# DelphinusLab/halo2-gpu-specific

Measured on AMD Instinct MI355X. Metric: NTT Fr-ops/s @ k=24 (forward+inverse 2^24 BN254 Fr NTT; MSM G1-adds/s under 'msm'), higher is better.
Workload: dtype u32x8 (254-bit Montgomery, integer)

## Files before the change

halo2-gpu-specific_amd/csrc/ntt.hip:

```cpp
#include <algorithm>
#include <cstdlib>
#include <memory>
#include <utility>

#include "common.hpp"
#include "ntt.hpp"
#include "ntt_pass.hpp"

namespace h2 {

void ntt_split(uint32_t log_n, std::vector<uint32_t>& bits) {
    bits.clear();
    if (log_n == 0) return;
    const uint32_t rem = log_n % 8, q = log_n / 8;
    static const bool nine = !(getenv("H2_NTT_NINE") && atoi(getenv("H2_NTT_NINE")) == 0);
    if (nine && q >= rem && (rem == 1 || (rem == 2 && log_n <= 18))) {
        for (uint32_t p = 0; p < q - rem; p++) bits.push_back(8);
        for (uint32_t p = 0; p < rem; p++) bits.push_back(9);
        return;
    }
    if (rem) bits.push_back(rem);
    for (uint32_t p = 0; p < q; p++) bits.push_back(8);
}

// ... 11 lines not shown
    sh.fixed = sh.radix4 && B == 8 && log_c == 2 && threads == 256;
    return sh;
}

std::vector<NttPass> ntt_schedule(uint32_t log_n) {
    std::vector<uint32_t> bits;
    ntt_split(log_n, bits);
    if (bits.empty()) bits.push_back(0);
    std::vector<NttPass> sched;
    uint32_t consumed = 0;
    for (size_t p = 0; p < bits.size(); p++) {
        NttPass ps{};
        ps.B = bits[p];
        ps.t_log = consumed;
        ps.s_log = log_n - consumed - ps.B;
        ps.last = p + 1 == bits.size();
        ps.shape = pass_shape(log_n, ps.B, ps.last ? ps.t_log : ps.s_log);
        sched.push_back(ps);
        consumed += ps.B;
    }
    return sched;
}

static uint32_t pass_zskip(uint32_t L, const NttPass& ps, uint32_t in_len) {
    static const bool no_zskip = getenv("H2_NTT_NO_ZSKIP") != nullptr;
    if (ps.t_log != 0 || ps.last || !in_len || in_len >= (1u << L) || (in_len & (in_len - 1)) != 0 || no_zskip) return 0;
    uint32_t z = 0;
    while ((in_len << z) < (1u << L)) z++;
    return z < ps.B ? z : ps.B;
}

static NttKernel pass_kernel(const NttPass& ps, uint32_t zskip) {
    if (!ps.shape.radix4) return NK_R2;
    const bool dp = !ps.last;
    if (ps.shape.fixed && zskip == 0) return dp ? NK_PASS8_DP : NK_PASS8;
    return dp ? NK_R4_DP : NK_R4;
}

size_t ntt_shape_query(uint32_t log_n, uint32_t in_log, uint32_t* out, size_t cap) {
    if (log_n == 0) return 0;
    const std::vector<NttPass> sched = ntt_schedule(log_n);
    for (size_t p = 0; p < sched.size() && p < cap; p++) {
        const NttPass& ps = sched[p];
        const uint32_t zskip = pass_zskip(log_n, ps, 1u << in_log);
        const uint32_t row[7] = {ps.B, ps.shape.log_c, ps.shape.threads, ps.shape.radix4, ps.shape.fixed, zskip,
                                 (uint32_t)pass_kernel(ps, zskip)};
        for (int i = 0; i < 7; i++) out[7 * p + i] = row[i];
    }
    return sched.size();
}

static std::string plan_key(uint32_t log_n, const uint64_t omega[4]) {
    char buf[128];
    snprintf(buf, sizeof buf, "%u:%016llx%016llx%016llx%016llx", log_n, (unsigned long long)omega[3],
             (unsigned long long)omega[2], (unsigned long long)omega[1], (unsigned long long)omega[0]);
    return buf;
}

static std::string fr_key(const Fr& v) {
    char buf[72];
    snprintf(buf, sizeof buf, "%08x%08x%08x%08x%08x%08x%08x%08x", v.l[7], v.l[6], v.l[5], v.l[4], v.l[3], v.l[2], v.l[1], v.l[0]);
    return buf;
}

Fr fr_from_u64x4(const uint64_t v[4]) {
    Fr r;
    for (int i = 0; i < 4; i++) {
        r.l[2 * i] = (uint32_t)v[i];
        r.l[2 * i + 1] = (uint32_t)(v[i] >> 32);
// ... 150 lines not shown
        ntt_fill_scaled(block.p, pl->tw_hi, d, cnt, stream);
        return block.publish(cnt * sizeof(Fr), stream);
    };
    return table_get(pl->cache, pl->scaled_hi, fr_key(d), build, [](std::vector<Fr*>&) {});
}

NttTablePin ntt_scale_table(NttPlan* pl, const Fr& g, const Fr* d, hipStream_t stream) {
    auto build = [&]() -> NttTable {
        const uint32_t n = 1u << pl->log_n;
        const uint32_t lo_count = n < (1u << LO_BITS) ? n : (1u << LO_BITS);
        const uint32_t hi_count = pl->log_n > LO_BITS ? (n >> LO_BITS) : 1u;
        const size_t bytes = ((size_t)(1u << LO_BITS) + hi_count) * sizeof(Fr);
        TableBlock block;
        H2_HIP(hipMalloc(&block.p, bytes));
        Fr* const hi = block.p + (1u << LO_BITS);
        ntt_fill_pow(block.p, g, 1u, lo_count, 0u, stream);
        ntt_fill_pow(hi, g, 1u << LO_BITS, hi_count, 0u, stream);
        if (d) ntt_fill_scaled(hi, hi, *d, hi_count, stream);
        return block.publish(bytes, stream);
    };
    auto admit = [&](std::vector<Fr*>& gone) {
        while (pl->scale_tabs.size() >= NttPlan::SCALE_TABS_MAX) {
            const auto lru = lru_idle(pl->scale_tabs);
            if (lru == pl->scale_tabs.end()) break;
            gone.push_back(lru->second.ptr);
            pl->scale_tabs.erase(lru);
        }
    };
    return table_get(pl->cache, pl->scale_tabs, d ? fr_key(g) + '*' + fr_key(*d) : fr_key(g) + '.', build, admit);
}

static void free_plan(NttPlan* pl) {
    if (pl->tables) (void)hipFree(pl->tables);
    for (const Fr* t : pl->tw_direct)
        if (t) (void)hipFree(const_cast<Fr*>(t));
    for (NttTableMap* map : {&pl->scaled_hi, &pl->scale_tabs, &pl->last_direct})
        for (auto& kv : *map) (void)hipFree(kv.second.ptr);
    delete pl;
}

static size_t plan_bytes(NttPlan* pl, bool* pinned = nullptr) {
    size_t bytes = pl->table_bytes;
    for (NttTableMap* map : {&pl->scaled_hi, &pl->scale_tabs, &pl->last_direct})
        for (auto& kv : *map) {
            bytes += kv.second.bytes;
            if (pinned && kv.second.users != 0) *pinned = true;
        }
    return bytes;
}

size_t ntt_plan_bytes(DeviceCtx* ctx) {
    NttCache* c = ctx->shared->ntt;
    std::lock_guard<std::mutex> g(c->mu);
    size_t bytes = 0;
    for (auto& kv : c->plans) bytes += plan_bytes(kv.second);
    return bytes;
}

void ntt_release_idle_plans(DeviceCtx* ctx) {
    NttCache* c = ctx->shared->ntt;
    std::vector<NttPlan*> gone;
    {
        std::lock_guard<std::mutex> g(c->mu);
        for (auto it = c->plans.begin(); it != c->plans.end();) {
            NttPlan* pl = it->second;
            bool busy = pl->users.load() != 0;
            plan_bytes(pl, &busy);
// ... 24 lines not shown
    };
    {
        std::lock_guard<std::mutex> g(c->mu);
        if (NttPlan* found = pin()) return PlanRef(found);
    }

    std::unique_ptr<NttPlan, void (*)(NttPlan*)> pl(new NttPlan(), free_plan);
    pl->cache = c;
    pl->log_n = log_n;
    pl->sched = ntt_schedule(log_n);
    const Fr w = pl->w = fr_from_u64x4(omega);
    const uint32_t n = 1u << log_n;
    const uint32_t lo_count = n < (1u << LO_BITS) ? n : (1u << LO_BITS);
    const uint32_t hi_count = log_n > LO_BITS ? (n >> LO_BITS) : 0;
    auto bfly_entries = [](const NttPass& ps) { return ((1u << ps.B) >> 1) * (ps.shape.radix4 ? 2u : 1u); };
    auto chunk_entries = [](const NttPass& ps) { return ps.shape.fixed ? ((1u << ps.B) >> 1) * TW_CHUNK_FR : 0u; };
    size_t total = lo_count + hi_count;
    for (const NttPass& ps : pl->sched) total += bfly_entries(ps) + chunk_entries(ps);
    H2_HIP(hipMalloc(&pl->tables, total * sizeof(Fr)));
    pl->table_bytes = total * sizeof(Fr);
    pl->tw_lo = pl->tables;
    pl->tw_hi = pl->tables + lo_count;
    ntt_fill_pow(pl->tables, w, 1u, lo_count, 0u, stream);
    ntt_fill_pow(pl->tables + lo_count, w, 1u << LO_BITS, hi_count, 0u, stream);
    Fr* next = pl->tables + lo_count + hi_count;
    for (const NttPass& ps : pl->sched) {
        const uint32_t half = (1u << ps.B) >> 1, form = ps.shape.radix4 ? 1u : 0u;
        ntt_fill_pow(next, w, n >> ps.B, half, form, stream);
        pl->tw_bfly.push_back(next);
        next += bfly_entries(ps);
        if (ps.shape.fixed) ntt_fill_pow(next, w, n >> ps.B, half, 2u, stream);
        pl->tw_chunk.push_back(ps.shape.fixed ? next : nullptr);
        next += chunk_entries(ps);
        Fr* direct = nullptr;
        if (ps.t_log != 0 && !ps.last && ps.B + ps.t_log <= 16) {
            const uint32_t cnt = 1u << (ps.B + ps.t_log);
            const size_t bytes = (size_t)cnt * sizeof(Fr) * (form ? 2 : 1);
            H2_HIP(hipMalloc(&direct, bytes));
            pl->table_bytes += bytes;
        }
        pl->tw_direct.push_back(direct);
        if (direct) ntt_fill_direct(direct, w, ps.t_log, ps.s_log, log_n, 1u << (ps.B + ps.t_log), form, stream);
    }
    H2_HIP(hipGetLastError());
    H2_HIP(hipStreamSynchronize(stream));
    std::lock_guard<std::mutex> g(c->mu);
    if (NttPlan* raced = pin()) return PlanRef(raced);
    c->plans[key] = pl.get();
    pl.release();
    return PlanRef(pin());
}

static void set_scale3(PassArgs& a, const Fr* pre3, const Fr* post3) {
    a.has_pre3 = pre3 != nullptr;
    a.has_post3 = post3 != nullptr;
    a.post3_uniform = post3 && fp_eq(post3[0], post3[1]) && fp_eq(post3[0], post3[2]);
    for (int i = 0; i < 3; i++) {
        if (pre3) a.pre3[i] = pre3[i];
        if (post3) a.post3[i] = post3[i];
    }
}

void ntt_run(DeviceCtx* ctx, NttPlan* pl, const Fr* src, Fr* dst, Fr* tmp, uint32_t in_len, const Fr* pre3,
             const Fr* post3, hipStream_t stream, const Fr* scale_tab, uint32_t scale_mode) {
    ntt_run_many(ctx, pl, &src, &dst, &tmp, 1, in_len, pre3, post3, stream, scale_tab, scale_mode);
}

static PassArgs pass_args(const NttPlan* pl, size_t p, const Fr* const* srcs, Fr* const* dsts, Fr* const* tmps, uint32_t cnt,
                          uint32_t in_len, const Fr* pre3, const Fr* post3, const Fr* scale_tab, uint32_t scale_mode) {
    const NttPass& ps = pl->sched[p];
    const bool first = p == 0, chain = pl->sched.size() >= 2;
    PassArgs a{};
    a.in = first ? srcs[0] : tmps[0];
    a.out = ps.last ? dsts[0] : tmps[0];
    if (cnt > 1) {
        a.batch = cnt;
        for (uint32_t i = 0; i < cnt; i++) {
            Fr* const work_i = chain ? tmps[i] : nullptr;
            a.in_b[i] = first ? srcs[i] : work_i;
            a.out_b[i] = ps.last ? dsts[i] : work_i;
        }
    }
    a.tw_bfly = pl->tw_bfly[p];
    a.tw_chunk = pl->tw_chunk[p];
    a.tw_lo = pl->tw_lo;
    a.tw_hi = pl->tw_hi;
    a.tw_direct = pl->tw_direct[p];
    set_scale3(a, first ? pre3 : nullptr, ps.last ? post3 : nullptr);
    a.log_n = pl->log_n;
    a.B = ps.B;
    a.s_log = ps.s_log;
    a.t_log = ps.t_log;
    a.nprev = (uint32_t)p;
    for (size_t q = 0; q < p; q++) {
        a.prevB[q] = pl->sched[q].B;
        a.prevT[q] = pl->sched[q].t_log;
    }
    a.is_last = ps.last ? 1 : 0;
    a.in_len = first ? in_len : (1u << pl->log_n);
    a.log_c = ps.shape.log_c;
    a.sc_lo = scale_tab;
    a.sc_hi = scale_tab ? scale_tab + (1u << LO_BITS) : nullptr;
    a.scale_mode = (scale_tab && ((scale_mode == 1u && first) || (scale_mode == 2u && ps.last))) ? scale_mode : 0u;
    a.zskip = pass_zskip(pl->log_n, ps, in_len);
    a.radix4 = ps.shape.radix4 ? 1u : 0u;
    return a;
}

static void ntt_run_chunk(DeviceCtx* ctx, NttPlan* pl, const Fr* const* srcs, Fr* const* dsts, Fr* const* tmps, uint32_t cnt,
                          uint32_t in_len, const Fr* pre3, const Fr* post3, hipStream_t stream, const Fr* scale_tab,
                          uint32_t scale_mode) {
    for (size_t p = 0; p < pl->sched.size(); p++) {
        const NttPass& ps = pl->sched[p];
        PassArgs a = pass_args(pl, p, srcs, dsts, tmps, cnt, in_len, pre3, post3, scale_tab, scale_mode);
        NttTablePin scaled_hi, last_tab;
        if (ps.last && p > 0) {
            if (a.post3_uniform && pl->log_n > LO_BITS) {
                scaled_hi = scaled_hi_table(pl, post3[0], stream);
                a.tw_hi = scaled_hi.get();
                a.hi_scaled = 1;
            }
            last_tab = last_table(ctx, pl, ps.B, a.hi_scaled ? &post3[0] : nullptr, stream);
            if (last_tab.get()) {
                a.tw_direct = last_tab.get();
                a.direct_kmajor = 1;
            }
        }
        ntt_pass_launch(ctx->device, pass_kernel(ps, a.zskip), a, cnt, ps.shape.threads, stream);
    }
    H2_HIP(hipGetLastError());
}

void ntt_run_many(DeviceCtx* ctx, NttPlan* pl, const Fr* const* srcs, Fr* const* dsts, Fr* const* tmps, size_t count,
                  uint32_t in_len, const Fr* pre3, const Fr* post3, hipStream_t stream, const Fr* scale_tab,
                  uint32_t scale_mode) {
    for (size_t c0 = 0; c0 < count; c0 += NTT_BATCH_MAX) {
        const uint32_t cnt = (uint32_t)std::min<size_t>(NTT_BATCH_MAX, count - c0);
        ntt_run_chunk(ctx, pl, srcs + c0, dsts + c0, tmps + c0, cnt, in_len, pre3, post3, stream, scale_tab, scale_mode);
    }
}

}
```

halo2-gpu-specific_amd/csrc/ntt.hpp:

```cpp
#pragma once
#include <atomic>
#include <vector>

#include "common.hpp"

namespace h2 {

struct PassShape {
    uint32_t log_c, threads;
    bool radix4;
    bool fixed;
};
struct NttPass {
    uint32_t B;
    uint32_t t_log;
    uint32_t s_log;
    bool last;
    PassShape shape;
};
void ntt_split(uint32_t log_n, std::vector<uint32_t>& bits);
std::vector<NttPass> ntt_schedule(uint32_t log_n);

struct NttPlan;
struct NttTable {
    Fr* ptr = nullptr;
    size_t bytes = 0;
    uint64_t last_use = 0;
    int users = 0;
};
using NttTableMap = std::map<std::string, NttTable>;

struct NttCache {
    std::mutex mu;
    std::map<std::string, NttPlan*> plans;
    size_t last_table_bytes = 0;
    uint64_t clock = 0;
};

struct NttPlan {
    NttCache* cache = nullptr;
    uint32_t log_n = 0;
    Fr w;
    std::vector<NttPass> sched;
    Fr* tables = nullptr;
    const Fr* tw_lo = nullptr;
    const Fr* tw_hi = nullptr;
    std::vector<const Fr*> tw_bfly;
    std::vector<const Fr*> tw_chunk;
    std::vector<const Fr*> tw_direct;
    size_t table_bytes = 0;
    NttTableMap scaled_hi;
    static constexpr size_t SCALE_TABS_MAX = 32;
    NttTableMap scale_tabs;
    NttTableMap last_direct;
    std::map<std::string, int> last_misses;
    std::atomic<int> users{0};
    uint64_t last_use = 0;
};

struct PlanRef {
    NttPlan* pl = nullptr;
    PlanRef() = default;
    explicit PlanRef(NttPlan* p) : pl(p) {}
    PlanRef(PlanRef&& o) noexcept : pl(o.pl) { o.pl = nullptr; }
    PlanRef& operator=(PlanRef&& o) noexcept {
        std::swap(pl, o.pl);
        return *this;
    }
    ~PlanRef() {
        if (pl) pl->users.fetch_sub(1);
    }
    NttPlan* operator->() const { return pl; }
    NttPlan* get() const { return pl; }
};

struct NttTablePin {
    NttCache* cache = nullptr;
    NttTable* tab = nullptr;
    NttTablePin() = default;
    NttTablePin(NttCache* c, NttTable* t) : cache(c), tab(t) {}
    NttTablePin(NttTablePin&& o) noexcept : cache(o.cache), tab(o.tab) { o.tab = nullptr; }
    NttTablePin& operator=(NttTablePin&& o) noexcept {
// ... 29 lines not shown
```

halo2-gpu-specific_amd/csrc/ntt_pass.hip:

```cpp
#include "ntt_pass.hpp"

namespace h2 {

__device__ __forceinline__ void tw_store(Fr* out, uint32_t i, const Fr& w_mont, uint32_t pair) {
    if (!pair) {
        fp_store(out + i, w_mont);
        return;
    }
    if (pair == 2) {
        TwChunk t;
        fp_chunk_table(w_mont, t);
        uint4* const q = reinterpret_cast<uint4*>(out) + (size_t)i * TW_CHUNK_Q;
#pragma unroll
        for (uint32_t k = 0; k < TW_CHUNK_Q; k++) q[k] = make_uint4(t.w[4 * k], t.w[4 * k + 1], t.w[4 * k + 2], t.w[4 * k + 3]);
        return;
    }
    Fr w, q;
    fp_const_pair(w_mont, w, q);
    fp_store(out + 2 * (size_t)i, w);
    fp_store(out + 2 * (size_t)i + 1, q);
}

__global__ void __launch_bounds__(256) k_pow_table(Fr* out, Fr base, uint32_t mul, uint32_t count, uint32_t pair) {
    uint32_t i = blockIdx.x * blockDim.x + threadIdx.x;
    if (i >= count) return;
    tw_store(out, i, fp_pow_u32(base, i * mul), pair);
}

__global__ void __launch_bounds__(256) k_direct_table(Fr* out, Fr base, uint32_t kbits, uint32_t s_log, uint32_t log_n,
                                                      uint32_t count, uint32_t pair) {
    uint32_t i = blockIdx.x * blockDim.x + threadIdx.x;
    if (i >= count) return;
// ... 30 lines not shown
    }
    return K;
}
__device__ __forceinline__ uint32_t K_to_hi(uint32_t K, const PassArgs& a) {
    uint32_t hi = 0;
    for (uint32_t q = 0; q < a.nprev; q++) {
        uint32_t d = (K >> a.prevT[q]) & ((1u << a.prevB[q]) - 1);
        hi = (hi << a.prevB[q]) | d;
    }
    return hi;
}

__device__ __forceinline__ Fr twiddle_pow(const PassArgs& a, uint32_t e) {
    if (a.log_n <= LO_BITS) return fp_load(a.tw_lo + e);
    Fr lo = fp_load(a.tw_lo + (e & ((1u << LO_BITS) - 1)));
    Fr hi = fp_load(a.tw_hi + (e >> LO_BITS));
    return fp_mul(lo, hi);
}

extern __shared__ __attribute__((aligned(16))) uint4 h2_smem[];

__device__ __forceinline__ Fr lds_get(const uint4* lo, const uint4* hi, uint32_t i) {
    uint4 a = lo[i], b = hi[i];
    Fr r;
    r.l[0] = a.x; r.l[1] = a.y; r.l[2] = a.z; r.l[3] = a.w;
    r.l[4] = b.x; r.l[5] = b.y; r.l[6] = b.z; r.l[7] = b.w;
    return r;
}
__device__ __forceinline__ void lds_put(uint4* lo, uint4* hi, uint32_t i, const Fr& v) {
    lo[i] = make_uint4(v.l[0], v.l[1], v.l[2], v.l[3]);
    hi[i] = make_uint4(v.l[4], v.l[5], v.l[6], v.l[7]);
}

template <bool RADIX4, bool DP = false>
__global__ void __launch_bounds__(512, 4) k_ntt_pass(PassArgs a) {
    constexpr bool CW = RADIX4;
    static_assert(!DP || CW, "pairs in tw_direct only next to pairs in tw_bfly");
    auto tmul = [](const Fr& x, const Fr& w) -> Fr { return fp_mul_wide(x, w); };
    const uint32_t B = a.B, R = 1u << B, log_c = a.log_c, C = 1u << log_c;
    const uint32_t zskip = a.zskip;
    uint4* t_lo = h2_smem;
    uint4* t_hi = t_lo + (R << log_c);
    uint4* w_lo = t_hi + (R << log_c);
    uint4* w_hi = w_lo + (R >> 1) + (CW ? 0 : 1);
    uint4* q_lo = w_hi + (R >> 1);
    uint4* q_hi = q_lo + (R >> 1);
    struct Tw {
        Fr w, q;
    };
    auto tw_get = [&](uint32_t i) __attribute__((always_inline)) -> Tw {
        Tw t;
        t.w = lds_get(w_lo, w_hi, i);
        if constexpr (CW) t.q = lds_get(q_lo, q_hi, i);
        return t;
    };
    auto bmul = [](const Fr& x, const Tw& t) __attribute__((always_inline)) -> Fr {
        if constexpr (CW) return fp_mul_const(x, t.w, t.q);
        else return fp_mul_wide(x, t.w);
    };
    const uint32_t nthreads = blockDim.x;
    const uint32_t tid = threadIdx.x;
    const Fr* const in_p = a.batch ? a.in_b[blockIdx.y] : a.in;
    Fr* const out_p = a.batch ? a.out_b[blockIdx.y] : a.out;
    const uint32_t n_mask = (a.log_n >= 32) ? 0xffffffffu : ((1u << a.log_n) - 1);

    for (uint32_t i = tid; i < (R >> 1); i += nthreads) {
        if constexpr (CW) {
            lds_put(w_lo, w_hi, i, fp_load(a.tw_bfly + 2 * i));
            lds_put(q_lo, q_hi, i, fp_load(a.tw_bfly + 2 * i + 1));
        } else {
            lds_put(w_lo, w_hi, i, fp_load(a.tw_bfly + i));
        }
    }

    const uint32_t tile_id = blockIdx.x;
    const uint32_t total = R << log_c;

    uint32_t base = 0, K_uniform = 0;
    const uint32_t S = 1u << a.s_log;
    if (!a.is_last) {
        uint32_t chunks_per_hi = S >> log_c;
        uint32_t hi = tile_id / chunks_per_hi, lo0 = (tile_id % chunks_per_hi) << log_c;
        base = (hi << (B + a.s_log)) + lo0;
        K_uniform = hi_to_K(hi, a);
    }

    constexpr uint32_t NE = RADIX4 ? 4 : 2;
    for (uint32_t e0 = tid; e0 < total; e0 += NE * nthreads) {
        uint32_t rho[NE], col[NE], idx[NE], Kk[NE];
        bool live[NE];
        Fr x[NE];
#pragma unroll
        for (uint32_t q = 0; q < NE; q++) {
            const uint32_t e = e0 + q * nthreads;
            if (!a.is_last) {
                col[q] = e & (C - 1);
                rho[q] = (e >> log_c) & (R - 1);
                idx[q] = base + (rho[q] << a.s_log) + col[q];
                Kk[q] = K_uniform;
            } else {
                rho[q] = e & (R - 1);
                col[q] = (e >> B) & (C - 1);
                Kk[q] = (tile_id << log_c) + col[q];
                idx[q] = (K_to_hi(Kk[q], a) << B) + rho[q];
            }
            live[q] = e < total && !(zskip && rho[q] >= (R >> zskip));
        }
#pragma unroll
        for (uint32_t q = 0; q < NE; q++) {
            x[q] = fp_zero<FrParams>();
            if (live[q] && idx[q] < a.in_len) x[q] = fp_load(in_p + idx[q]);
        }
        if (a.has_pre3) {
#pragma unroll
            for (uint32_t q = 0; q < NE; q++) {
                const uint32_t m = idx[q] % 3;
                Fr w;
#pragma unroll
                for (int l = 0; l < 8; l++) w.l[l] = m == 1 ? a.pre3[1].l[l] : a.pre3[2].l[l];
                if (m != 0) x[q] = tmul(x[q], w);
            }
        }
        const bool pre_scale = a.scale_mode == 1u && a.nprev == 0;
        if (a.nprev != 0 || pre_scale) {
            if (a.tw_direct != nullptr && !pre_scale) {
#pragma unroll
                for (uint32_t q0 = 0; q0 < NE; q0 += 2) {
                    if constexpr (DP) {
#pragma unroll
                        for (uint32_t q = q0; q < q0 + 2; q++) {
                            const size_t at = a.direct_kmajor ? ((Kk[q] << B) | rho[q]) : ((rho[q] << a.t_log) | Kk[q]);
                            const Fr w = fp_load(a.tw_direct + 2 * at), wq = fp_load(a.tw_direct + 2 * at + 1);
                            x[q] = fp_mul_const(x[q], w, wq);
                        }
                    } else {
                        Fr w[2];
#pragma unroll
                        for (uint32_t q = 0; q < 2; q++)
                            w[q] = fp_load(a.tw_direct + (a.direct_kmajor ? ((Kk[q0 + q] << B) | rho[q0 + q]) : ((rho[q0 + q] << a.t_log) | Kk[q0 + q])));
#pragma unroll
                        for (uint32_t q = 0; q < 2; q++) x[q0 + q] = tmul(x[q0 + q], w[q]);
                    }
                }
            } else if (a.log_n <= LO_BITS && !pre_scale) {
#pragma unroll
                for (uint32_t q = 0; q < NE; q++) {
                    const uint32_t ex = (uint32_t)(((uint64_t)rho[q] * Kk[q]) << a.s_log) & n_mask;
                    x[q] = tmul(x[q], fp_load(a.tw_lo + ex));
                }
            } else {
                const Fr* const two_lo = pre_scale ? a.sc_lo : a.tw_lo;
                const Fr* const two_hi = pre_scale ? a.sc_hi : a.tw_hi;
#pragma unroll
                for (uint32_t q0 = 0; q0 < NE; q0 += 2) {
                    Fr wl[2], wh[2];
#pragma unroll
                    for (uint32_t q = 0; q < 2; q++) {
                        const uint32_t ex = pre_scale ? (idx[q0 + q] & n_mask)
                                                      : ((uint32_t)(((uint64_t)rho[q0 + q] * Kk[q0 + q]) << a.s_log) & n_mask);
                        wl[q] = fp_load(two_lo + (ex & ((1u << LO_BITS) - 1)));
                        wh[q] = fp_load(two_hi + (ex >> LO_BITS));
                    }
#pragma unroll
                    for (uint32_t q = 0; q < 2; q++) x[q0 + q] = tmul(x[q0 + q], fp_mul(wl[q], wh[q]));
                }
            }
        }
#pragma unroll
        for (uint32_t q = 0; q < NE; q++) {
            const uint32_t e = e0 + q * nthreads;
            const uint32_t r_q = a.is_last ? (e & (R - 1)) : ((e >> log_c) & (R - 1));
            const uint32_t c_q = a.is_last ? ((e >> B) & (C - 1)) : (e & (C - 1));
            if (e >= total || (zskip && r_q >= (R >> zskip))) continue;
            if (zskip) {
                for (uint32_t m = 0; m < (1u << zskip); m++) lds_put(t_lo, t_hi, ((bitrev(r_q, B) | m) << log_c) + c_q, x[q]);
            } else {
                lds_put(t_lo, t_hi, (bitrev(r_q, B) << log_c) + c_q, x[q]);
            }
        }
    }
    __syncthreads();

    uint32_t s0 = zskip;
    if constexpr (RADIX4) {
        const uint32_t nunits = total >> 2;
        auto round4 = [&](const uint32_t s) __attribute__((always_inline)) {
            const uint32_t h = 1u << s;
            const uint32_t log_per = (B - 2 + log_c) - s;
            const bool by_r = s != 0 && log_per >= 6 && (nthreads & 63) == 0;
            for (uint32_t t = tid; t < nunits; t += nthreads) {
                uint32_t c, r, p;
                if (by_r) {
                    r = t >> log_per;
                    const uint32_t j = t & ((1u << log_per) - 1);
                    c = j & (C - 1);
                    p = ((j >> log_c) << (s + 2)) | r;
                } else {
                    c = t & (C - 1);
                    const uint32_t b = t >> log_c;
                    r = b & (h - 1);
                    p = ((b >> s) << (s + 2)) | r;
                }
                const uint32_t i0 = (p << log_c) + c, step = h << log_c;
                Fr x0 = lds_get(t_lo, t_hi, i0), x1 = lds_get(t_lo, t_hi, i0 + step);
                Fr x2 = lds_get(t_lo, t_hi, i0 + 2 * step), x3 = lds_get(t_lo, t_hi, i0 + 3 * step);
// ... 27 lines not shown
        const uint32_t log_per = (B - 1 + log_c) - s;
        const bool by_r = s != 0 && log_per >= 6 && (nthreads & 63) == 0;
        for (uint32_t t = tid; t < nbf; t += nthreads) {
            uint32_t c, r, i;
            if (by_r) {
                r = t >> log_per;
                uint32_t j = t & ((1u << log_per) - 1);
                c = j & (C - 1);
                i = ((j >> log_c) << (s + 1)) | r;
            } else {
                c = t & (C - 1);
                uint32_t b = t >> log_c;
                r = b & (h - 1);
                i = ((b >> s) << (s + 1)) | r;
            }
            const uint32_t iu = (i << log_c) + c, iv = ((i + h) << log_c) + c;
            Fr u = lds_get(t_lo, t_hi, iu), v = lds_get(t_lo, t_hi, iv);
            const bool skip = s == 0 || (by_r && r == 0);
            u = fp_lazy_red2p(u);
            v = skip ? fp_lazy_red2p(v) : bmul(v, tw_get(r << (B - 1 - s)));
            lds_put(t_lo, t_hi, iu, fp_lazy_add(u, v));
            lds_put(t_lo, t_hi, iv, fp_lazy_sub(u, v));
        }
        __syncthreads();
    }

    for (uint32_t e0 = tid; e0 < total; e0 += NE * nthreads) {
        Fr y[NE];
        uint32_t idx[NE];
#pragma unroll
        for (uint32_t q = 0; q < NE; q++) {
            const uint32_t e = e0 + q * nthreads;
            const uint32_t c = e & (C - 1), k = (e >> log_c) & (R - 1);
            if (!a.is_last)
                idx[q] = base + (k << a.s_log) + c;
            else
                idx[q] = ((tile_id << log_c) + c) + (k << a.t_log);
            y[q] = lds_get(t_lo, t_hi, (k << log_c) + c);
        }
        if (a.is_last && a.scale_mode == 2u) {
#pragma unroll
            for (uint32_t q = 0; q < NE; q++) {
                const uint32_t i = idx[q] & n_mask;
                const Fr w = fp_mul(fp_load(a.sc_lo + (i & ((1u << LO_BITS) - 1))), fp_load(a.sc_hi + (i >> LO_BITS)));
                y[q] = fp_reduce_once(fp_mul_wide(y[q], w));
            }
        } else if (a.is_last && a.has_post3 && !a.hi_scaled) {
#pragma unroll
            for (uint32_t q = 0; q < NE; q++) {
                const uint32_t m = idx[q] % 3;
                Fr w;
#pragma unroll
                for (int l = 0; l < 8; l++) w.l[l] = m == 0 ? a.post3[0].l[l] : (m == 1 ? a.post3[1].l[l] : a.post3[2].l[l]);
                y[q] = fp_reduce_once(fp_mul_wide(y[q], w));
            }
        } else if (a.is_last) {
#pragma unroll
            for (uint32_t q = 0; q < NE; q++) y[q] = fp_lazy_canon(y[q]);
        }
#pragma unroll
        for (uint32_t q = 0; q < NE; q++)
            if (e0 + q * nthreads < total) fp_store(out_p + idx[q], y[q]);
    }
}

static constexpr uint32_t PASS8_TW_LDS = 32;
static constexpr uint32_t PASS8_LDS = ((256u << 2) * 2 + PASS8_TW_LDS * TW_CHUNK_Q) * sizeof(uint4);
static_assert(4 * PASS8_LDS <= 160u * 1024, "four workgroups of k_ntt_pass8 per CU");
template <bool DP>
__global__ void __launch_bounds__(256, 4) k_ntt_pass8(PassArgs a) {
    constexpr uint32_t B = 8, R = 1u << B, log_c = 2, C = 1u << log_c;
    auto tmul = [](const Fr& x, const Fr& w) -> Fr { return fp_mul_wide(x, w); };
    uint4* t_lo = h2_smem;
    uint4* t_hi = t_lo + (R << log_c);
    uint4* w_pl = t_hi + (R << log_c);
    const uint4* const tw_tab = reinterpret_cast<const uint4*>(a.tw_chunk);
    using Tw = TwChunk;
    auto tw_unpack = [](Tw& t, const uint32_t k, const uint4 v) __attribute__((always_inline)) {
        t.w[4 * k] = v.x; t.w[4 * k + 1] = v.y; t.w[4 * k + 2] = v.z; t.w[4 * k + 3] = v.w;
    };
    static_assert((R >> 1) / PASS8_TW_LDS == 4, "the stage pairs before the last read the indices that are multiples of 4");
    auto tw_get = [&](const uint32_t i, const bool mem) __attribute__((always_inline)) -> Tw {
        Tw t;
#pragma unroll
        for (uint32_t k = 0; k < TW_CHUNK_Q; k++)
            tw_unpack(t, k, mem ? tw_tab[(size_t)i * TW_CHUNK_Q + k] : w_pl[k * PASS8_TW_LDS + (i >> 2)]);
        return t;
    };
    auto bmul = [](const Fr& x, const Tw& t) __attribute__((always_inline)) -> Fr { return fp_mul_chunk(x, t); };
    auto unit4 = [&](Fr& x0, Fr& x1, Fr& x2, Fr& x3, const uint32_t s, const uint32_t r, const bool unit, const Tw* w3 = nullptr) __attribute__((always_inline)) {
        const uint32_t h = 1u << s;
        const bool mem = s == B - 2;
        x0 = fp_lazy_red2p(x0);
        x2 = fp_lazy_red2p(x2);
        if (!unit) {
            const Tw wa = tw_get(r << (B - 1 - s), mem);
            x1 = bmul(x1, wa);
            x3 = bmul(x3, wa);
        } else {
            x1 = fp_lazy_red2p(x1);
            x3 = fp_lazy_red2p(x3);
        }
        const Fr y0 = fp_lazy_add_red(x0, x1), y1 = fp_lazy_sub_red(x0, x1);
// ... 8 lines not shown
    auto unit_of = [](const uint32_t tid, const uint32_t s, uint32_t& i0, uint32_t& r, bool& unit) __attribute__((always_inline)) {
        const uint32_t h = 1u << s, log_per = (B - 2 + log_c) - s;
        const bool by_r = s != 0 && log_per >= 6;
        uint32_t c, p;
        if (by_r) {
            r = tid >> log_per;
            const uint32_t j = tid & ((1u << log_per) - 1);
            c = j & (C - 1);
            p = ((j >> log_c) << (s + 2)) | r;
        } else {
            c = tid & (C - 1);
            const uint32_t b = tid >> log_c;
            r = b & (h - 1);
            p = ((b >> s) << (s + 2)) | r;
        }
        i0 = (p << log_c) + c;
        unit = s == 0 || (by_r && r == 0);
    };
    const uint32_t tid = threadIdx.x;
    auto round4 = [&](const uint32_t s) __attribute__((always_inline)) {
        uint32_t i0, r;
        bool unit;
        unit_of(tid, s, i0, r, unit);
        const uint32_t step = (1u << s) << log_c;
        Fr x0 = lds_get(t_lo, t_hi, i0), x1 = lds_get(t_lo, t_hi, i0 + step);
        Fr x2 = lds_get(t_lo, t_hi, i0 + 2 * step), x3 = lds_get(t_lo, t_hi, i0 + 3 * step);
        unit4(x0, x1, x2, x3, s, r, unit);
        lds_put(t_lo, t_hi, i0, x0);
        lds_put(t_lo, t_hi, i0 + 2 * step, x2);
        lds_put(t_lo, t_hi, i0 + step, x1);
        lds_put(t_lo, t_hi, i0 + 3 * step, x3);
        __syncthreads();
    };
    const bool is_last = DP ? false : a.is_last != 0;
    const uint32_t n_mask = (a.log_n >= 32) ? 0xffffffffu : ((1u << a.log_n) - 1);

#pragma unroll
    for (uint32_t g = tid; g < PASS8_TW_LDS * TW_CHUNK_Q; g += 256)
        w_pl[(g % TW_CHUNK_Q) * PASS8_TW_LDS + g / TW_CHUNK_Q] = tw_tab[(size_t)(g / TW_CHUNK_Q) * 4 * TW_CHUNK_Q + g % TW_CHUNK_Q];

    Tw tw64;
#pragma unroll
    for (uint32_t k = 0; k < TW_CHUNK_Q; k++) tw_unpack(tw64, k, tw_tab[(R >> 2) * TW_CHUNK_Q + k]);

    constexpr uint32_t NE = 4;
    {
        const uint32_t tile_id = blockIdx.x;
        const Fr* const in_p = a.batch ? a.in_b[blockIdx.y] : a.in;
        Fr* const out_p = a.batch ? a.out_b[blockIdx.y] : a.out;
        uint32_t base = 0, K_uniform = 0;
        if (!is_last) {
            const uint32_t chunks_per_hi = (1u << a.s_log) >> log_c;
            const uint32_t hi = tile_id / chunks_per_hi, lo0 = (tile_id % chunks_per_hi) << log_c;
            base = (hi << (B + a.s_log)) + lo0;
            K_uniform = hi_to_K(hi, a);
        }

        {
            uint32_t rho[NE], col[NE], idx[NE], Kk[NE];
            Fr x[NE];
#pragma unroll
            for (uint32_t q = 0; q < NE; q++) {
                if (!is_last) {
                    col[q] = tid & (C - 1);
                    rho[q] = bitrev(tid >> log_c, B - 2) + (q << (B - 2));
                    idx[q] = base + (rho[q] << a.s_log) + col[q];
                    Kk[q] = K_uniform;
                } else {
                    rho[q] = (tid & 63) + (q << (B - 2));
                    col[q] = tid >> 6;
                    Kk[q] = (tile_id << log_c) + col[q];
                    idx[q] = (K_to_hi(Kk[q], a) << B) + rho[q];
                }
            }
#pragma unroll
            for (uint32_t q = 0; q < NE; q++) {
                x[q] = fp_zero<FrParams>();
                if (idx[q] < a.in_len) x[q] = fp_load(in_p + idx[q]);
            }
            if (a.has_pre3) {
#pragma unroll
                for (uint32_t q = 0; q < NE; q++) {
                    const uint32_t m = idx[q] % 3;
                    Fr w;
#pragma unroll
                    for (int l = 0; l < 8; l++) w.l[l] = m == 1 ? a.pre3[1].l[l] : a.pre3[2].l[l];
                    if (m != 0) x[q] = tmul(x[q], w);
                }
            }
            const bool pre_scale = a.scale_mode == 1u && a.nprev == 0;
            if (a.nprev != 0 || pre_scale) {
                if (a.tw_direct != nullptr && !pre_scale) {
#pragma unroll
                    for (uint32_t q0 = 0; q0 < NE; q0 += 2) {
                        if constexpr (DP) {
#pragma unroll
                            for (uint32_t q = q0; q < q0 + 2; q++) {
                                const size_t at = a.direct_kmajor ? ((Kk[q] << B) | rho[q]) : ((rho[q] << a.t_log) | Kk[q]);
                                const Fr w = fp_load(a.tw_direct + 2 * at), wq = fp_load(a.tw_direct + 2 * at + 1);
                                x[q] = fp_mul_const(x[q], w, wq);
                            }
                        } else {
                            Fr w[2];
#pragma unroll
                            for (uint32_t q = 0; q < 2; q++)
                                w[q] = fp_load(a.tw_direct + (a.direct_kmajor ? ((Kk[q0 + q] << B) | rho[q0 + q]) : ((rho[q0 + q] << a.t_log) | Kk[q0 + q])));
#pragma unroll
                            for (uint32_t q = 0; q < 2; q++) x[q0 + q] = tmul(x[q0 + q], w[q]);
                        }
                    }
                } else if (a.log_n <= LO_BITS && !pre_scale) {
#pragma unroll
                    for (uint32_t q = 0; q < NE; q++) {
                        const uint32_t ex = (uint32_t)(((uint64_t)rho[q] * Kk[q]) << a.s_log) & n_mask;
                        x[q] = tmul(x[q], fp_load(a.tw_lo + ex));
                    }
                } else {
                    const Fr* const two_lo = pre_scale ? a.sc_lo : a.tw_lo;
                    const Fr* const two_hi = pre_scale ? a.sc_hi : a.tw_hi;
#pragma unroll
                    for (uint32_t q0 = 0; q0 < NE; q0 += 2) {
                        Fr wl[2], wh[2];
#pragma unroll
                        for (uint32_t q = 0; q < 2; q++) {
                            const uint32_t ex = pre_scale ? (idx[q0 + q] & n_mask)
                                                          : ((uint32_t)(((uint64_t)rho[q0 + q] * Kk[q0 + q]) << a.s_log) & n_mask);
                            wl[q] = fp_load(two_lo + (ex & ((1u << LO_BITS) - 1)));
                            wh[q] = fp_load(two_hi + (ex >> LO_BITS));
                        }
#pragma unroll
                        for (uint32_t q = 0; q < 2; q++) x[q0 + q] = tmul(x[q0 + q], fp_mul(wl[q], wh[q]));
                    }
                }
            }
            const uint32_t b = is_last ? bitrev(tid & 63, B - 2) : (tid >> log_c);
            const uint32_t i0 = (b << (2 + log_c)) + (is_last ? (tid >> 6) : (tid & (C - 1)));
            unit4(x[0], x[2], x[1], x[3], 0, 0, true, &tw64);
            lds_put(t_lo, t_hi, i0, x[0]);
            lds_put(t_lo, t_hi, i0 + 2 * C, x[1]);
            lds_put(t_lo, t_hi, i0 + C, x[2]);
            lds_put(t_lo, t_hi, i0 + 3 * C, x[3]);
        }
// ... 8 lines not shown
            unit_of(tid, 6, i0, r, unit);
#pragma unroll
            for (uint32_t q = 0; q < NE; q++) y[q] = lds_get(t_lo, t_hi, i0 + q * (R << log_c) / NE);
            unit4(y[0], y[1], y[2], y[3], 6, r, unit);
        }
        uint32_t idx[NE];
#pragma unroll
        for (uint32_t q = 0; q < NE; q++) {
            const uint32_t c = tid & (C - 1), k = (tid >> log_c) + q * (R / NE);
            if (!is_last)
                idx[q] = base + (k << a.s_log) + c;
            else
                idx[q] = ((tile_id << log_c) + c) + (k << a.t_log);
        }
        if (is_last && a.scale_mode == 2u) {
#pragma unroll
            for (uint32_t q = 0; q < NE; q++) {
                const uint32_t i = idx[q] & n_mask;
                const Fr w = fp_mul(fp_load(a.sc_lo + (i & ((1u << LO_BITS) - 1))), fp_load(a.sc_hi + (i >> LO_BITS)));
                y[q] = fp_reduce_once(fp_mul_wide(y[q], w));
            }
        } else if (is_last && a.has_post3 && !a.hi_scaled) {
#pragma unroll
            for (uint32_t q = 0; q < NE; q++) {
                const uint32_t m = idx[q] % 3;
                Fr w;
#pragma unroll
                for (int l = 0; l < 8; l++) w.l[l] = m == 0 ? a.post3[0].l[l] : (m == 1 ? a.post3[1].l[l] : a.post3[2].l[l]);
                y[q] = fp_reduce_once(fp_mul_wide(y[q], w));
            }
        } else if (is_last) {
#pragma unroll
            for (uint32_t q = 0; q < NE; q++) y[q] = fp_lazy_canon(y[q]);
        }
#pragma unroll
        for (uint32_t q = 0; q < NE; q++) fp_store(out_p + idx[q], y[q]);
    }
}

using PassFn = void (*)(PassArgs);
static const PassFn pass_fn[H2_NTT_KERNEL_COUNT] = {
    k_ntt_pass8<true>,
    k_ntt_pass8<false>,
    k_ntt_pass<true, true>,
    k_ntt_pass<true, false>,
    k_ntt_pass<false>,
};

void ntt_pass_launch(int device, NttKernel kernel, const PassArgs& a, uint32_t cnt, uint32_t threads, hipStream_t stream) {
    const uint32_t R = 1u << a.B, C = 1u << a.log_c;
    const uint32_t ntiles = (1u << a.log_n) / (R * C);
    const size_t lds = kernel != NK_R2 ? ((size_t)R * C + R) * sizeof(Fr) : ((size_t)R * C + (R >> 1) + 2) * sizeof(Fr);
    if (lds > 64 * 1024) {
        static bool raised[64] = {};
        if (device < 0 || device >= 64 || !raised[device]) {
            for (NttKernel k : {NK_R4_DP, NK_R4, NK_R2})
                H2_HIP(hipFuncSetAttribute((const void*)pass_fn[k], hipFuncAttributeMaxDynamicSharedMemorySize, 160 * 1024));
            if (device >= 0 && device < 64) raised[device] = true;
        }
    }
    const bool pass8 = kernel == NK_PASS8_DP || kernel == NK_PASS8;
    hipLaunchKernelGGL(pass_fn[kernel], dim3(ntiles, cnt), dim3(threads), pass8 ? (size_t)PASS8_LDS : lds, stream, a);
}

static dim3 fill_grid(uint32_t count) { return dim3((count + 255) / 256); }

void ntt_fill_pow(Fr* out, const Fr& base, uint32_t mul, uint32_t count, uint32_t form, hipStream_t stream) {
    if (count) hipLaunchKernelGGL(k_pow_table, fill_grid(count), dim3(256), 0, stream, out, base, mul, count, form);
}

void ntt_fill_direct(Fr* out, const Fr& base, uint32_t kbits, uint32_t s_log, uint32_t log_n, uint32_t count, uint32_t form,
                     hipStream_t stream) {
    hipLaunchKernelGGL(k_direct_table, fill_grid(count), dim3(256), 0, stream, out, base, kbits, s_log, log_n, count, form);
}

void ntt_fill_last(Fr* out, const Fr& base, uint32_t bits, uint32_t log_n, const Fr* d, hipStream_t stream) {
    hipLaunchKernelGGL(k_last_table, fill_grid(1u << log_n), dim3(256), 0, stream, out, base, bits, log_n, d ? *d : base,
                       d ? 1u : 0u, 0u);
}

void ntt_fill_scaled(Fr* out, const Fr* in, const Fr& d, uint32_t count, hipStream_t stream) {
    hipLaunchKernelGGL(k_scale_table, fill_grid(count), dim3(256), 0, stream, out, in, d, count);
}

}
```

halo2-gpu-specific_amd/csrc/ntt_pass.hpp:

```cpp
#pragma once
#include "common.hpp"

namespace h2 {

static constexpr int NTT_BATCH_MAX = 16;
static constexpr int LO_BITS = 12;

using TwChunk = FpChunk<2>;
static constexpr uint32_t TW_CHUNK_FR = sizeof(TwChunk) / sizeof(Fr);
static constexpr uint32_t TW_CHUNK_Q = sizeof(TwChunk) / sizeof(uint4);

struct PassArgs {
    const Fr* in;
    Fr* out;
    const Fr* tw_bfly;
    const Fr* tw_chunk;
    const Fr* tw_lo;
    const Fr* tw_hi;
    const Fr* tw_direct;
    uint32_t direct_kmajor;
    uint32_t hi_scaled;
    Fr pre3[3];
    Fr post3[3];
    uint32_t has_pre3, has_post3, post3_uniform;
    uint32_t log_n, B, s_log, t_log;
    uint32_t nprev;
    uint32_t prevB[4];
    uint32_t prevT[4];
    uint32_t is_last, in_len, log_c;
    const Fr* sc_lo;
    const Fr* sc_hi;
    uint32_t scale_mode;
    uint32_t batch;
    const Fr* in_b[NTT_BATCH_MAX];
    Fr* out_b[NTT_BATCH_MAX];
    uint32_t zskip;
    uint32_t radix4;
};

enum NttKernel : uint32_t {
    NK_PASS8_DP = H2_NTT_KERNEL_PASS8_DP,
    NK_PASS8 = H2_NTT_KERNEL_PASS8,
    NK_R4_DP = H2_NTT_KERNEL_R4_DP,
    NK_R4 = H2_NTT_KERNEL_R4,
    NK_R2 = H2_NTT_KERNEL_R2,
};

void ntt_pass_launch(int device, NttKernel kernel, const PassArgs& a, uint32_t cnt, uint32_t threads, hipStream_t stream);

void ntt_fill_pow(Fr* out, const Fr& base, uint32_t mul, uint32_t count, uint32_t form, hipStream_t stream);
void ntt_fill_direct(Fr* out, const Fr& base, uint32_t kbits, uint32_t s_log, uint32_t log_n, uint32_t count, uint32_t form,
                     hipStream_t stream);
void ntt_fill_last(Fr* out, const Fr& base, uint32_t bits, uint32_t log_n, const Fr* d, hipStream_t stream);
// ... 4 lines not shown
```

Before: 426.0 billion.

## Apply next pass's inter-pass twiddles at store time of the previous NTT pass

Instead of the next pass loading per-element direct twiddles after reading its input, the producing pass now multiplies each output by the next pass's twiddle before storing it, using a chunked (precomputed-constant) table layout and a new store-twiddle kernel variant. The consuming pass skips its twiddle multiply when flagged as already applied. The aim is to move the twiddle load and multiply out of the next pass's load phase and into a store phase that may overlap better. The cost is a separate kernel instantiation and a larger table per entry, and the index mapping between passes must be correct.

Result: faster. 436.3 billion (median of 6 runs) (+2.4%).

```diff
diff --git a/halo2-gpu-specific_amd/csrc/ntt.hip b/halo2-gpu-specific_amd/csrc/ntt.hip
--- a/halo2-gpu-specific_amd/csrc/ntt.hip
+++ b/halo2-gpu-specific_amd/csrc/ntt.hip
@@ -67,9 +67,8 @@
 
 static NttKernel pass_kernel(const NttPass& ps, uint32_t zskip) {
     if (!ps.shape.radix4) return NK_R2;
-    const bool dp = !ps.last;
-    if (ps.shape.fixed && zskip == 0) return dp ? NK_PASS8_DP : NK_PASS8;
-    return dp ? NK_R4_DP : NK_R4;
+    if (ps.shape.fixed && zskip == 0) return ps.last ? NK_PASS8 : NK_PASS8_DP;
+    return ps.last ? NK_R4 : NK_R4_DP;
 }
 
 size_t ntt_shape_query(uint32_t log_n, uint32_t in_log, uint32_t* out, size_t cap) {
@@ -286,7 +285,7 @@
 
 static void free_plan(NttPlan* pl) {
     if (pl->tables) (void)hipFree(pl->tables);
-    for (const Fr* t : pl->tw_direct)
+    for (const Fr* t : pl->tw_inter)
         if (t) (void)hipFree(const_cast<Fr*>(t));
     for (NttTableMap* map : {&pl->scaled_hi, &pl->scale_tabs, &pl->last_direct})
         for (auto& kv : *map) (void)hipFree(kv.second.ptr);
@@ -377,15 +376,15 @@
         if (ps.shape.fixed) ntt_fill_pow(next, w, n >> ps.B, half, 2u, stream);
         pl->tw_chunk.push_back(ps.shape.fixed ? next : nullptr);
         next += chunk_entries(ps);
-        Fr* direct = nullptr;
+        Fr* tab = nullptr;
         if (ps.t_log != 0 && !ps.last && ps.B + ps.t_log <= 16) {
             const uint32_t cnt = 1u << (ps.B + ps.t_log);
-            const size_t bytes = (size_t)cnt * sizeof(Fr) * (form ? 2 : 1);
-            H2_HIP(hipMalloc(&direct, bytes));
+            const size_t bytes = (size_t)cnt * sizeof(TwChunk);
+            H2_HIP(hipMalloc(&tab, bytes));
             pl->table_bytes += bytes;
         }
-        pl->tw_direct.push_back(direct);
-        if (direct) ntt_fill_direct(direct, w, ps.t_log, ps.s_log, log_n, 1u << (ps.B + ps.t_log), form, stream);
+        pl->tw_inter.push_back(tab);
+        if (tab) ntt_fill_direct(tab, w, ps.t_log, ps.s_log, log_n, 1u << (ps.B + ps.t_log), 2u, stream);
     }
     H2_HIP(hipGetLastError());
     H2_HIP(hipStreamSynchronize(stream));
@@ -430,7 +429,14 @@
     a.tw_chunk = pl->tw_chunk[p];
     a.tw_lo = pl->tw_lo;
     a.tw_hi = pl->tw_hi;
-    a.tw_direct = pl->tw_direct[p];
+    a.tw_applied = pl->tw_inter[p] != nullptr;
+    if (!ps.last && pl->tw_inter[p + 1]) {
+        const NttPass& nx = pl->sched[p + 1];
+        a.nx_tab = pl->tw_inter[p + 1];
+        a.nx_s_log = nx.s_log;
+        a.nx_B = nx.B;
+        a.nx_t_log = nx.t_log;
+    }
     set_scale3(a, first ? pre3 : nullptr, ps.last ? post3 : nullptr);
     a.log_n = pl->log_n;
     a.B = ps.B;
@@ -466,10 +472,7 @@
                 a.hi_scaled = 1;
             }
             last_tab = last_table(ctx, pl, ps.B, a.hi_scaled ? &post3[0] : nullptr, stream);
-            if (last_tab.get()) {
-                a.tw_direct = last_tab.get();
-                a.direct_kmajor = 1;
-            }
+            a.tw_direct = last_tab.get();
         }
         ntt_pass_launch(ctx->device, pass_kernel(ps, a.zskip), a, cnt, ps.shape.threads, stream);
     }
diff --git a/halo2-gpu-specific_amd/csrc/ntt.hpp b/halo2-gpu-specific_amd/csrc/ntt.hpp
--- a/halo2-gpu-specific_amd/csrc/ntt.hpp
+++ b/halo2-gpu-specific_amd/csrc/ntt.hpp
@@ -47,7 +47,7 @@
     const Fr* tw_hi = nullptr;
     std::vector<const Fr*> tw_bfly;
     std::vector<const Fr*> tw_chunk;
-    std::vector<const Fr*> tw_direct;
+    std::vector<const Fr*> tw_inter;
     size_t table_bytes = 0;
     NttTableMap scaled_hi;
     static constexpr size_t SCALE_TABS_MAX = 32;
diff --git a/halo2-gpu-specific_amd/csrc/ntt_pass.hip b/halo2-gpu-specific_amd/csrc/ntt_pass.hip
--- a/halo2-gpu-specific_amd/csrc/ntt_pass.hip
+++ b/halo2-gpu-specific_amd/csrc/ntt_pass.hip
@@ -1,3 +1,5 @@
+#include <stdexcept>
+
 #include "ntt_pass.hpp"
 
 namespace h2 {
@@ -94,10 +96,22 @@
     hi[i] = make_uint4(v.l[4], v.l[5], v.l[6], v.l[7]);
 }
 
-template <bool RADIX4, bool DP = false>
+__device__ __forceinline__ Fr store_twiddle(const PassArgs& a, const Fr& y, const uint32_t entry) {
+    const uint4* const q = reinterpret_cast<const uint4*>(a.nx_tab) + (size_t)entry * TW_CHUNK_Q;
+    TwChunk t;
+#pragma unroll
+    for (uint32_t k = 0; k < TW_CHUNK_Q; k++) {
+        const uint4 v = q[k];
+        t.w[4 * k] = v.x; t.w[4 * k + 1] = v.y; t.w[4 * k + 2] = v.z; t.w[4 * k + 3] = v.w;
+    }
+    return fp_mul_chunk(y, t);
+}
+
+template <bool RADIX4, bool NLAST = false, bool ST = false>
 __global__ void __launch_bounds__(512, 4) k_ntt_pass(PassArgs a) {
     constexpr bool CW = RADIX4;
-    static_assert(!DP || CW, "pairs in tw_direct only next to pairs in tw_bfly");
+    static_assert(!ST || NLAST || !RADIX4, "a last pass stores the transform's output");
+    const bool is_last = NLAST ? false : a.is_last != 0;
     auto tmul = [](const Fr& x, const Fr& w) -> Fr { return fp_mul_wide(x, w); };
     const uint32_t B = a.B, R = 1u << B, log_c = a.log_c, C = 1u << log_c;
     const uint32_t zskip = a.zskip;
@@ -140,7 +154,7 @@
 
     uint32_t base = 0, K_uniform = 0;
     const uint32_t S = 1u << a.s_log;
-    if (!a.is_last) {
+    if (!is_last) {
         uint32_t chunks_per_hi = S >> log_c;
         uint32_t hi = tile_id / chunks_per_hi, lo0 = (tile_id % chunks_per_hi) << log_c;
         base = (hi << (B + a.s_log)) + lo0;
@@ -155,7 +169,7 @@
 #pragma unroll
         for (uint32_t q = 0; q < NE; q++) {
             const uint32_t e = e0 + q * nthreads;
-            if (!a.is_last) {
+            if (!is_last) {
                 col[q] = e & (C - 1);
                 rho[q] = (e >> log_c) & (R - 1);
                 idx[q] = base + (rho[q] << a.s_log) + col[q];
@@ -184,25 +198,15 @@
             }
         }
         const bool pre_scale = a.scale_mode == 1u && a.nprev == 0;
-        if (a.nprev != 0 || pre_scale) {
-            if (a.tw_direct != nullptr && !pre_scale) {
+        if ((a.nprev != 0 && !a.tw_applied) || pre_scale) {
+            if (!NLAST && a.tw_direct != nullptr && !pre_scale) {
 #pragma unroll
                 for (uint32_t q0 = 0; q0 < NE; q0 += 2) {
-                    if constexpr (DP) {
-#pragma unroll
-                        for (uint32_t q = q0; q < q0 + 2; q++) {
-                            const size_t at = a.direct_kmajor ? ((Kk[q] << B) | rho[q]) : ((rho[q] << a.t_log) | Kk[q]);
-                            const Fr w = fp_load(a.tw_direct + 2 * at), wq = fp_load(a.tw_direct + 2 * at + 1);
-                            x[q] = fp_mul_const(x[q], w, wq);
-                        }
-                    } else {
-                        Fr w[2];
-#pragma unroll
-                        for (uint32_t q = 0; q < 2; q++)
-                            w[q] = fp_load(a.tw_direct + (a.direct_kmajor ? ((Kk[q0 + q] << B) | rho[q0 + q]) : ((rho[q0 + q] << a.t_log) | Kk[q0 + q])));
-#pragma unroll
-                        for (uint32_t q = 0; q < 2; q++) x[q0 + q] = tmul(x[q0 + q], w[q]);
-                    }
+                    Fr w[2];
+#pragma unroll
+                    for (uint32_t q = 0; q < 2; q++) w[q] = fp_load(a.tw_direct + ((Kk[q0 + q] << B) | rho[q0 + q]));
+#pragma unroll
+                    for (uint32_t q = 0; q < 2; q++) x[q0 + q] = tmul(x[q0 + q], w[q]);
                 }
             } else if (a.log_n <= LO_BITS && !pre_scale) {
 #pragma unroll
@@ -231,8 +235,8 @@
 #pragma unroll
         for (uint32_t q = 0; q < NE; q++) {
             const uint32_t e = e0 + q * nthreads;
-            const uint32_t r_q = a.is_last ? (e & (R - 1)) : ((e >> log_c) & (R - 1));
-            const uint32_t c_q = a.is_last ? ((e >> B) & (C - 1)) : (e & (C - 1));
+            const uint32_t r_q = is_last ? (e & (R - 1)) : ((e >> log_c) & (R - 1));
+            const uint32_t c_q = is_last ? ((e >> B) & (C - 1)) : (e & (C - 1));
             if (e >= total || (zskip && r_q >= (R >> zskip))) continue;
             if (zskip) {
                 for (uint32_t m = 0; m < (1u << zskip); m++) lds_put(t_lo, t_hi, ((bitrev(r_q, B) | m) << log_c) + c_q, x[q]);
@@ -326,20 +330,20 @@
         for (uint32_t q = 0; q < NE; q++) {
             const uint32_t e = e0 + q * nthreads;
             const uint32_t c = e & (C - 1), k = (e >> log_c) & (R - 1);
-            if (!a.is_last)
+            if (!is_last)
                 idx[q] = base + (k << a.s_log) + c;
             else
                 idx[q] = ((tile_id << log_c) + c) + (k << a.t_log);
             y[q] = lds_get(t_lo, t_hi, (k << log_c) + c);
         }
-        if (a.is_last && a.scale_mode == 2u) {
+        if (is_last && a.scale_mode == 2u) {
 #pragma unroll
             for (uint32_t q = 0; q < NE; q++) {
                 const uint32_t i = idx[q] & n_mask;
                 const Fr w = fp_mul(fp_load(a.sc_lo + (i & ((1u << LO_BITS) - 1))), fp_load(a.sc_hi + (i >> LO_BITS)));
                 y[q] = fp_reduce_once(fp_mul_wide(y[q], w));
             }
-        } else if (a.is_last && a.has_post3 && !a.hi_scaled) {
+        } else if (is_last && a.has_post3 && !a.hi_scaled) {
 #pragma unroll
             for (uint32_t q = 0; q < NE; q++) {
                 const uint32_t m = idx[q] % 3;
@@ -348,9 +352,18 @@
                 for (int l = 0; l < 8; l++) w.l[l] = m == 0 ? a.post3[0].l[l] : (m == 1 ? a.post3[1].l[l] : a.post3[2].l[l]);
                 y[q] = fp_reduce_once(fp_mul_wide(y[q], w));
             }
-        } else if (a.is_last) {
+        } else if (is_last) {
 #pragma unroll
             for (uint32_t q = 0; q < NE; q++) y[q] = fp_lazy_canon(y[q]);
+        }
+        if constexpr (ST) {
+#pragma unroll
+            for (uint32_t q = 0; q < NE; q++) {
+                const uint32_t e = e0 + q * nthreads;
+                const uint32_t rho_n = (idx[q] >> a.nx_s_log) & ((1u << a.nx_B) - 1);
+                const uint32_t K_n = K_uniform | (((e >> log_c) & (R - 1)) << a.t_log);
+                if (e < total) y[q] = store_twiddle(a, y[q], (rho_n << a.nx_t_log) | K_n);
+            }
         }
 #pragma unroll
         for (uint32_t q = 0; q < NE; q++)
@@ -361,8 +374,9 @@
 static constexpr uint32_t PASS8_TW_LDS = 32;
 static constexpr uint32_t PASS8_LDS = ((256u << 2) * 2 + PASS8_TW_LDS * TW_CHUNK_Q) * sizeof(uint4);
 static_assert(4 * PASS8_LDS <= 160u * 1024, "four workgroups of k_ntt_pass8 per CU");
-template <bool DP>
+template <bool NLAST, bool ST = false>
 __global__ void __launch_bounds__(256, 4) k_ntt_pass8(PassArgs a) {
+    static_assert(!ST || NLAST, "a last pass stores the transform's output");
     constexpr uint32_t B = 8, R = 1u << B, log_c = 2, C = 1u << log_c;
     auto tmul = [](const Fr& x, const Fr& w) -> Fr { return fp_mul_wide(x, w); };
     uint4* t_lo = h2_smem;
@@ -437,7 +451,7 @@
         lds_put(t_lo, t_hi, i0 + 3 * step, x3);
         __syncthreads();
     };
-    const bool is_last = DP ? false : a.is_last != 0;
+    const bool is_last = NLAST ? false : a.is_last != 0;
     const uint32_t n_mask = (a.log_n >= 32) ? 0xffffffffu : ((1u << a.log_n) - 1);
 
 #pragma unroll
@@ -494,25 +508,15 @@
                 }
             }
             const bool pre_scale = a.scale_mode == 1u && a.nprev == 0;
-            if (a.nprev != 0 || pre_scale) {
-                if (a.tw_direct != nullptr && !pre_scale) {
+            if ((a.nprev != 0 && !a.tw_applied) || pre_scale) {
+                if (!NLAST && a.tw_direct != nullptr && !pre_scale) {
 #pragma unroll
                     for (uint32_t q0 = 0; q0 < NE; q0 += 2) {
-                        if constexpr (DP) {
-#pragma unroll
-                            for (uint32_t q = q0; q < q0 + 2; q++) {
-                                const size_t at = a.direct_kmajor ? ((Kk[q] << B) | rho[q]) : ((rho[q] << a.t_log) | Kk[q]);
-                                const Fr w = fp_load(a.tw_direct + 2 * at), wq = fp_load(a.tw_direct + 2 * at + 1);
-                                x[q] = fp_mul_const(x[q], w, wq);
-                            }
-                        } else {
-                            Fr w[2];
-#pragma unroll
-                            for (uint32_t q = 0; q < 2; q++)
-                                w[q] = fp_load(a.tw_direct + (a.direct_kmajor ? ((Kk[q0 + q] << B) | rho[q0 + q]) : ((rho[q0 + q] << a.t_log) | Kk[q0 + q])));
-#pragma unroll
-                            for (uint32_t q = 0; q < 2; q++) x[q0 + q] = tmul(x[q0 + q], w[q]);
-                        }
+                        Fr w[2];
+#pragma unroll
+                        for (uint32_t q = 0; q < 2; q++) w[q] = fp_load(a.tw_direct + ((Kk[q0 + q] << B) | rho[q0 + q]));
+#pragma unroll
+                        for (uint32_t q = 0; q < 2; q++) x[q0 + q] = tmul(x[q0 + q], w[q]);
                     }
                 } else if (a.log_n <= LO_BITS && !pre_scale) {
 #pragma unroll
@@ -587,6 +591,14 @@
         } else if (is_last) {
 #pragma unroll
             for (uint32_t q = 0; q < NE; q++) y[q] = fp_lazy_canon(y[q]);
+        }
+        if constexpr (ST) {
+            const uint32_t rho_n = (base >> a.nx_s_log) & ((1u << a.nx_B) - 1);
+#pragma unroll
+            for (uint32_t q = 0; q < NE; q++) {
+                const uint32_t K_n = K_uniform | (((tid >> log_c) + q * (R / NE)) << a.t_log);
+                y[q] = store_twiddle(a, y[q], (rho_n << a.nx_t_log) | K_n);
+            }
         }
 #pragma unroll
         for (uint32_t q = 0; q < NE; q++) fp_store(out_p + idx[q], y[q]);
@@ -601,6 +613,9 @@
     k_ntt_pass<true, false>,
     k_ntt_pass<false>,
 };
+static const PassFn pass_fn_st[H2_NTT_KERNEL_COUNT] = {
+    k_ntt_pass8<true, true>, nullptr, k_ntt_pass<true, true, true>, nullptr, k_ntt_pass<false, false, true>,
+};
 
 void ntt_pass_launch(int device, NttKernel kernel, const PassArgs& a, uint32_t cnt, uint32_t threads, hipStream_t stream) {
     const uint32_t R = 1u << a.B, C = 1u << a.log_c;
@@ -609,13 +624,15 @@
     if (lds > 64 * 1024) {
         static bool raised[64] = {};
         if (device < 0 || device >= 64 || !raised[device]) {
-            for (NttKernel k : {NK_R4_DP, NK_R4, NK_R2})
-                H2_HIP(hipFuncSetAttribute((const void*)pass_fn[k], hipFuncAttributeMaxDynamicSharedMemorySize, 160 * 1024));
+            for (const PassFn f : {pass_fn[NK_R4_DP], pass_fn[NK_R4], pass_fn[NK_R2], pass_fn_st[NK_R4_DP], pass_fn_st[NK_R2]})
+                H2_HIP(hipFuncSetAttribute((const void*)f, hipFuncAttributeMaxDynamicSharedMemorySize, 160 * 1024));
             if (device >= 0 && device < 64) raised[device] = true;
         }
     }
     const bool pass8 = kernel == NK_PASS8_DP || kernel == NK_PASS8;
-    hipLaunchKernelGGL(pass_fn[kernel], dim3(ntiles, cnt), dim3(threads), pass8 ? (size_t)PASS8_LDS : lds, stream, a);
+    const PassFn fn = a.nx_tab ? pass_fn_st[kernel] : pass_fn[kernel];
+    if (!fn) throw std::runtime_error("ntt_pass_launch: a last pass has no next pass to multiply for");
+    hipLaunchKernelGGL(fn, dim3(ntiles, cnt), dim3(threads), pass8 ? (size_t)PASS8_LDS : lds, stream, a);
 }
 
 static dim3 fill_grid(uint32_t count) { return dim3((count + 255) / 256); }
diff --git a/halo2-gpu-specific_amd/csrc/ntt_pass.hpp b/halo2-gpu-specific_amd/csrc/ntt_pass.hpp
--- a/halo2-gpu-specific_amd/csrc/ntt_pass.hpp
+++ b/halo2-gpu-specific_amd/csrc/ntt_pass.hpp
@@ -18,7 +18,9 @@
     const Fr* tw_lo;
     const Fr* tw_hi;
     const Fr* tw_direct;
-    uint32_t direct_kmajor;
+    uint32_t tw_applied;
+    const Fr* nx_tab;
+    uint32_t nx_s_log, nx_B, nx_t_log;
     uint32_t hi_scaled;
     Fr pre3[3];
     Fr post3[3];
```
